# henriChevreux/distillation_trajectories

Measured on AMD Instinct MI355X. Metric: trajectory-timesteps/sec (B×T U-Net fwd) at 16×16 T=50, higher is better.
Workload: dtype f32 (fp32-accurate; convolutions: exact 3-plane bf16 operand split on bf16 MFMA with fp32 accumulate, or native fp32 MFMA, chosen per layer)

## Files before the change

distillation_trajectories_amd/csrc/dt_conv_strip.hip:

```cpp
#include <mutex>
#include <type_traits>

#include "dt_conv_epilogue.h"

namespace dt {

extern __shared__ __attribute__((aligned(16))) __bf16 strip_lds[];

template <int BM, int BN, int KC = 1, int WK = 1>
__global__ __launch_bounds__(256, KC == 1 ? 3 : 2) void conv_strip_bf16x6_kernel(const ConvParams p) {
  constexpr int WN = WK > 1 ? BN / 64 : (BM == 256 ? 1 : 2), WM = 4 / (WN * WK), NT = 256;
  constexpr int MI = BM / (32 * WM), NI = BN / (32 * WN);
  constexpr int KW = KC / WK;
  static_assert(KC % WK == 0 && MI * 32 * WM == BM && NI * 32 * WN == BN && (WK == 1 || (MI == 2 && NI == 2)), "wave layout");
  constexpr int PLANE_B = BN * 16, STAGE_B = 3 * PLANE_B;
  constexpr int AP = BM == 256 ? 3 : (KC == 4 ? 1 : 2);
  const int halo = strip_halo(p.W, BM);
  const int R = BM + 2 * halo;
  const int RZ = (R + 7) & ~7;
  const int PLANE_A = (RZ + 8) * 16;
  __bf16 *As = strip_lds;
  __bf16 *Bs = strip_lds + KC * 3 * PLANE_A;

  const int tid = threadIdx.x, lane = tid & 63;
  const int wave = __builtin_amdgcn_readfirstlane(tid >> 6);
  const int wk = wave % WK, wm = (wave / WK) / WN, wn = (wave / WK) % WN;
  const int half = lane >> 5, l31 = lane & 31;
  const int m0 = blockIdx.x * BM, n0 = blockIdx.y * BN;
  const int HW = p.H * p.W;
  const int CC = p.cin_p >> 4;

  bool s_in[AP], s_ok[AP], s_core[AP];
  int s_off[AP], s_off2[AP], s_offb[AP], s_lds[AP];
#pragma unroll
  for (int i = 0; i < AP; ++i) {
    const int item = tid + i * NT;
    const int srow = item >> 1, hh = item & 1;
    const int m = m0 - halo + srow;
    s_in[i] = item < 2 * R;
    s_ok[i] = s_in[i] && m >= 0 && m < p.M;
    s_core[i] = s_ok[i] && srow >= halo && srow < halo + BM;
    const int mm = s_ok[i] ? m : 0;
    s_off[i] = mm * p.cin_p + hh * 8;
    s_off2[i] = mm * p.cin2_p + hh * 8;
    s_offb[i] = mm * p.b_stride + hh * 8;
    s_lds[i] = srow * 16 + ((hh ^ ((srow >> 3) & 1)) << 3);
  }
  constexpr bool B_ALL = WK > 1 && BN * 4 == NT;
  constexpr int NB = B_ALL ? KC * 3 / 2 : KC * 3, SB = B_ALL ? 2 : 1;
  static_assert(!B_ALL || (KC * 3) % 2 == 0, "weight staging");
  const bool b_thread = B_ALL || tid < BN * 2;
  const int bt = B_ALL ? (tid & (BN * 2 - 1)) : tid, bsub = B_ALL ? tid / (BN * 2) : 0;
  const size_t w_plane = (size_t)p.n_p * 16;
  const __bf16 *wbase = reinterpret_cast<const __bf16 *>(p.w) + (size_t)n0 * 16 + bt * 8 + bsub * w_plane;
  const __bf16 *wbase2 = reinterpret_cast<const __bf16 *>(p.w2) + (size_t)n0 * 16 + bt * 8 + bsub * w_plane;
  const int b_lds = bsub * PLANE_B + bt * 8;

  int a_row[MI];
  unsigned a_mask[MI];
#pragma unroll
  for (int mi = 0; mi < MI; ++mi) {
    const int row_i = wm * (MI * 32) + mi * 32 + l31;
    const int m = m0 + row_i;
    a_row[mi] = row_i + halo;
    unsigned mask = 0;
    if (m < p.M) {
      const int rem = m % HW;
      const int y = rem / p.W, x = rem - y * p.W;
#pragma unroll
      for (int t = 0; t < 9; ++t) {
        const int yy = y + t / 3 - 1, xx = x + t % 3 - 1;
        if (yy >= 0 && yy < p.H && xx >= 0 && xx < p.W) mask |= 1u << t;
      }
    }
    a_mask[mi] = mask;
  }
  int b_frag[NI];
#pragma unroll
  for (int ni = 0; ni < NI; ++ni) {
    const int row = wn * (NI * 32) + ni * 32 + l31;
    b_frag[ni] = row * 16 + ((half ^ ((row >> 3) & 1)) << 3);
  }

  f32x16 acc[MI][NI];
#pragma unroll
  for (int mi = 0; mi < MI; ++mi)
#pragma unroll
    for (int ni = 0; ni < NI; ++ni)
#pragma unroll
      for (int r = 0; r < 16; ++r) acc[mi][ni][r] = 0.f;

  const int n_main = (CC + p.splits * KC - 1) / (p.splits * KC);
  const int cc0 = blockIdx.z * n_main * KC;
  const int CC2 = p.cin2_p >> 4;
  const int n_chunks = n_main + (p.in2 ? (CC2 + KC - 1) / KC : 0);

  f32x4 sa0[KC][AP], sa1[KC][AP];
  u32x4 rb[NB];
  auto load_strip = [&](int ch) __attribute__((always_inline)) {
#pragma unroll
    for (int kk = 0; kk < KC; ++kk)
#pragma unroll
    for (int i = 0; i < AP; ++i) {
      sa0[kk][i] = f32x4{0.f, 0.f, 0.f, 0.f}; sa1[kk][i] = sa0[kk][i];
      if (ch < n_main) {
        const int cc = cc0 + ch * KC + kk;
        if (s_ok[i] && cc < CC) {
          const float *src = (p.in_b && cc >= p.cc_a) ? p.in_b + s_offb[i] + (cc - p.cc_a) * 16 : p.in + s_off[i] + cc * 16;
          sa0[kk][i] = *reinterpret_cast<const f32x4 *>(src);
          sa1[kk][i] = *reinterpret_cast<const f32x4 *>(src + 4);
        }
      } else if (s_core[i] && (ch - n_main) * KC + kk < CC2) {
        const int c2 = (ch - n_main) * KC + kk;
        const float *src = (p.in2_b && c2 >= p.cc_a) ? p.in2_b + s_offb[i] + (c2 - p.cc_a) * 16 : p.in2 + s_off2[i] + c2 * 16;
        sa0[kk][i] = *reinterpret_cast<const f32x4 *>(src);
        sa1[kk][i] = *reinterpret_cast<const f32x4 *>(src + 4);
      }
    }
  };
  auto write_strip = [&]() __attribute__((always_inline)) {
#pragma unroll
    for (int kk = 0; kk < KC; ++kk)
#pragma unroll
    for (int i = 0; i < AP; ++i)
      if (s_in[i]) {
        bf16x8 p1, p2, p3;
        split8(sa0[kk][i], sa1[kk][i], p1, p2, p3);
        __bf16 *A = As + kk * 3 * PLANE_A;
        *reinterpret_cast<bf16x8 *>(A + s_lds[i]) = p1;
        *reinterpret_cast<bf16x8 *>(A + PLANE_A + s_lds[i]) = p2;
        *reinterpret_cast<bf16x8 *>(A + 2 * PLANE_A + s_lds[i]) = p3;
      }
  };
  const size_t tap_stride = (size_t)p.ccw * 3 * w_plane, group_stride = (size_t)KC * 3 * w_plane;
  const __bf16 *wrun = wbase + (size_t)cc0 * 3 * w_plane;
  enum { ADV_NONE = 0, ADV_TAP, ADV_GROUP, ADV_SKIP0, ADV_SKIP };
  auto load_b = [&](int adv) __attribute__((always_inline)) {
    if (adv == ADV_TAP) wrun += tap_stride;
    else if (adv == ADV_GROUP) wrun = wrun - 8 * tap_stride + group_stride;
    else if (adv == ADV_SKIP0) wrun = wbase2;
    else if (adv == ADV_SKIP) wrun += group_stride;
    if (b_thread) {
#pragma unroll
      for (int i = 0; i < NB; ++i)
        rb[i] = *reinterpret_cast<const u32x4 *>(wrun + (SB * i) * w_plane);
    }
  };
  auto write_b = [&](int stage) __attribute__((always_inline)) {
    if (b_thread) {
      __bf16 *B = Bs + stage * KC * STAGE_B;
#pragma unroll
      for (int i = 0; i < NB; ++i) *reinterpret_cast<u32x4 *>(B + (SB * i) * PLANE_B + b_lds) = rb[i];
    }
  };

  constexpr bool DB = WK > 1;
  bf16x8 fbn[KW][NI][3];
  auto load_bd = [&](int adv) __attribute__((always_inline)) {
    if (adv == ADV_TAP) wrun += tap_stride;
    else if (adv == ADV_GROUP) wrun = wrun - 8 * tap_stride + group_stride;
    else if (adv == ADV_SKIP0) wrun = wbase2;
    else if (adv == ADV_SKIP) wrun += group_stride;
    const __bf16 *wt = wrun - (bt * 8 + bsub * w_plane);
#pragma unroll
    for (int kw = 0; kw < KW; ++kw)
#pragma unroll
      for (int ni = 0; ni < NI; ++ni)
#pragma unroll
        for (int pl = 0; pl < 3; ++pl)
          fbn[kw][ni][pl] = *reinterpret_cast<const bf16x8 *>(wt + ((wk * KW + kw) * 3 + pl) * w_plane + b_frag[ni]);
  };

  load_strip(0);
  if (DB) load_bd(ADV_NONE); else load_b(ADV_NONE);
  if (tid < 48 * KC) *reinterpret_cast<u32x4 *>(As + (tid >> 4) * PLANE_A + RZ * 16 + (tid & 15) * 8) = u32x4{0u, 0u, 0u, 0u};
  write_strip();
  if (!DB) write_b(0);
  __syncthreads();

  int step = 0;
  bool stage_next_strip = true;
  auto do_step = [&](auto TT, int ch, bool first_tap, bool last_tap, bool next_chunk, int adv) __attribute__((always_inline)) {
    constexpr int tt = decltype(TT)::value;
    const bool more = !last_tap || next_chunk;
    if (first_tap && next_chunk && stage_next_strip) load_strip(ch + 1);
    bf16x8 fbc[KW][NI][3];
    if (DB) {
#pragma unroll
      for (int kw = 0; kw < KW; ++kw)
#pragma unroll
        for (int ni = 0; ni < NI; ++ni)
#pragma unroll
          for (int pl = 0; pl < 3; ++pl) fbc[kw][ni][pl] = fbn[kw][ni][pl];
      if (more) load_bd(adv);
    } else if (more) load_b(adv);
    {
      int wv = p.W;
      asm volatile("" : "+s"(wv));
      const int shift = (tt / 3 - 1) * wv + (tt % 3 - 1);
      int a_e[MI];
#pragma unroll
      for (int mi = 0; mi < MI; ++mi) {
        int row0 = a_row[mi];
        asm volatile("" : "+v"(row0));
        const int srow = row0 + shift;
        const int lrow = ((a_mask[mi] >> tt) & 1u) ? srow : RZ + (srow & 7);
        a_e[mi] = lrow * 16 + ((half ^ ((srow >> 3) & 1)) << 3);
      }
#pragma unroll
      for (int kw = 0; kw < KW; ++kw) {
        const int kk = wk * KW + kw;
        const __bf16 *A = As + kk * 3 * PLANE_A;
        const __bf16 *B = Bs + ((step & 1) * KC + kk) * STAGE_B;
        bf16x8 fb[NI][3];
#pragma unroll
        for (int ni = 0; ni < NI; ++ni)
#pragma unroll
          for (int pl = 0; pl < 3; ++pl)
            fb[ni][pl] = DB ? fbc[kw][ni][pl] : *reinterpret_cast<const bf16x8 *>(B + pl * PLANE_B + b_frag[ni]);
#pragma unroll
        for (int mi = 0; mi < MI; ++mi) {
          bf16x8 fa[3];
#pragma unroll
          for (int pl = 0; pl < 3; ++pl)
            fa[pl] = *reinterpret_cast<const bf16x8 *>(A + pl * PLANE_A + a_e[mi]);
#pragma unroll
          for (int ni = 0; ni < NI; ++ni) {
            f32x16 c = acc[mi][ni];
            c = __builtin_amdgcn_mfma_f32_32x32x16_bf16(fa[2], fb[ni][0], c, 0, 0, 0);
            c = __builtin_amdgcn_mfma_f32_32x32x16_bf16(fa[1], fb[ni][1], c, 0, 0, 0);
            c = __builtin_amdgcn_mfma_f32_32x32x16_bf16(fa[0], fb[ni][2], c, 0, 0, 0);
            c = __builtin_amdgcn_mfma_f32_32x32x16_bf16(fa[1], fb[ni][0], c, 0, 0, 0);
            c = __builtin_amdgcn_mfma_f32_32x32x16_bf16(fa[0], fb[ni][1], c, 0, 0, 0);
            c = __builtin_amdgcn_mfma_f32_32x32x16_bf16(fa[0], fb[ni][0], c, 0, 0, 0);
            acc[mi][ni] = c;
          }
        }
      }
    }
    if (!DB && more) write_b((step + 1) & 1);
    const bool restage = last_tap && next_chunk && stage_next_strip;
    if (restage) {
      __syncthreads();
      write_strip();
    }
    if (!DB || restage) __syncthreads();
    ++step;
  };

  constexpr bool DIRECT = MI * KW <= 2 && KC >= 2;
  f32x4 ga0[KW][MI][2], ga1[KW][MI][2];
  const int n_skip = p.in2 ? (CC2 + KC - 1) / KC : 0;
  auto load_a = [&](f32x4 (&g)[KW][MI][2], int s2) __attribute__((always_inline)) {
#pragma unroll
    for (int kw = 0; kw < KW; ++kw)
#pragma unroll
      for (int mi = 0; mi < MI; ++mi) {
        const int c2 = s2 * KC + wk * KW + kw;
        const int m = m0 + wm * (MI * 32) + mi * 32 + l31;
        g[kw][mi][0] = f32x4{0.f, 0.f, 0.f, 0.f}; g[kw][mi][1] = g[kw][mi][0];
        if (m < p.M && c2 < CC2) {
          const float *src = (p.in2_b && c2 >= p.cc_a) ? p.in2_b + (size_t)m * p.b_stride + (c2 - p.cc_a) * 16 + half * 8
                                                       : p.in2 + (size_t)m * p.cin2_p + c2 * 16 + half * 8;
          g[kw][mi][0] = *reinterpret_cast<const f32x4 *>(src);
          g[kw][mi][1] = *reinterpret_cast<const f32x4 *>(src + 4);
        }
      }
  };
  auto skip_step = [&](f32x4 (&g)[KW][MI][2], int s2) __attribute__((always_inline)) {
    const bool more = s2 + 1 < n_skip;
    bf16x8 fbc[KW][NI][3];
    if (DB) {
#pragma unroll
      for (int kw = 0; kw < KW; ++kw)
#pragma unroll
        for (int ni = 0; ni < NI; ++ni)
#pragma unroll
          for (int pl = 0; pl < 3; ++pl) fbc[kw][ni][pl] = fbn[kw][ni][pl];
      if (more) load_bd(ADV_SKIP);
    } else if (more) load_b(ADV_SKIP);
#pragma unroll
    for (int kw = 0; kw < KW; ++kw) {
      const int kk = wk * KW + kw;
      const __bf16 *B = Bs + ((step & 1) * KC + kk) * STAGE_B;
      bf16x8 fb[NI][3];
#pragma unroll
      for (int ni = 0; ni < NI; ++ni)
#pragma unroll
        for (int pl = 0; pl < 3; ++pl) fb[ni][pl] = DB ? fbc[kw][ni][pl] : *reinterpret_cast<const bf16x8 *>(B + pl * PLANE_B + b_frag[ni]);
#pragma unroll
      for (int mi = 0; mi < MI; ++mi) {
        bf16x8 fa[3];
        split8(g[kw][mi][0], g[kw][mi][1], fa[0], fa[1], fa[2]);
#pragma unroll
        for (int ni = 0; ni < NI; ++ni) {
          f32x16 c = acc[mi][ni];
          c = __builtin_amdgcn_mfma_f32_32x32x16_bf16(fa[2], fb[ni][0], c, 0, 0, 0);
          c = __builtin_amdgcn_mfma_f32_32x32x16_bf16(fa[1], fb[ni][1], c, 0, 0, 0);
          c = __builtin_amdgcn_mfma_f32_32x32x16_bf16(fa[0], fb[ni][2], c, 0, 0, 0);
          c = __builtin_amdgcn_mfma_f32_32x32x16_bf16(fa[1], fb[ni][0], c, 0, 0, 0);
          c = __builtin_amdgcn_mfma_f32_32x32x16_bf16(fa[0], fb[ni][1], c, 0, 0, 0);
          c = __builtin_amdgcn_mfma_f32_32x32x16_bf16(fa[0], fb[ni][0], c, 0, 0, 0);
          acc[mi][ni] = c;
        }
      }
    }
    if (s2 + 2 < n_skip) load_a(g, s2 + 2);
    if (!DB) {
      if (more) write_b((step + 1) & 1);
      __syncthreads();
    }
    ++step;
  };

  const int prio_grp = ((blockIdx.x + gridDim.x * (blockIdx.y + gridDim.y * blockIdx.z)) >> 8) & 1;
  const bool use_prio = gridDim.x * gridDim.y * gridDim.z <= 512;
  for (int ch = 0; ch < n_main; ++ch) {
    if (use_prio) {
      if ((ch ^ prio_grp) & 1) __builtin_amdgcn_s_setprio(1);
      else __builtin_amdgcn_s_setprio(0);
    }
    const bool next_chunk = ch + 1 < ((WK > 1 && p.in2) ? n_main : n_chunks);
    if (DIRECT && WK == 1 && p.in2 && ch + 1 == n_main) {
      stage_next_strip = false;
      load_a(ga0, 0);
      if (n_skip > 1) load_a(ga1, 1);
    }
    do_step(std::integral_constant<int, 0>{}, ch, true, false, next_chunk, ADV_TAP);
    do_step(std::integral_constant<int, 1>{}, ch, false, false, next_chunk, ADV_TAP);
    do_step(std::integral_constant<int, 2>{}, ch, false, false, next_chunk, ADV_TAP);
    do_step(std::integral_constant<int, 3>{}, ch, false, false, next_chunk, ADV_TAP);
    do_step(std::integral_constant<int, 4>{}, ch, false, false, next_chunk, ADV_TAP);
    do_step(std::integral_constant<int, 5>{}, ch, false, false, next_chunk, ADV_TAP);
    do_step(std::integral_constant<int, 6>{}, ch, false, false, next_chunk, ADV_TAP);
    do_step(std::integral_constant<int, 7>{}, ch, false, false, next_chunk, ADV_TAP);
    do_step(std::integral_constant<int, 8>{}, ch, false, true, next_chunk, ch + 1 < n_main ? ADV_GROUP : ADV_SKIP0);
    if (ch + 1 == n_main && p.in2) {
      if constexpr (WK == 1) {
        conv_midpoint<MI, NI>(p, acc, n0, wn, l31);
      } else {
        constexpr int P = BN + 4, COPY = WM * 32 * P;
        float *red = reinterpret_cast<float *>(strip_lds);
#pragma unroll
        for (int mi = 0; mi < MI; ++mi) {
          if (mi || DB) __syncthreads();
#pragma unroll
          for (int ni = 0; ni < NI; ++ni)
#pragma unroll
            for (int r = 0; r < 16; ++r)
              red[wk * COPY + (wm * 32 + 4 * half + (r & 3) + 8 * (r >> 2)) * P + wn * (NI * 32) + ni * 32 + l31] = acc[mi][ni][r];
          __syncthreads();
#pragma unroll
          for (int ni = 0; ni < NI; ++ni)
#pragma unroll
            for (int r = 0; r < 16; ++r) {
              const float *src = red + (wm * 32 + 4 * half + (r & 3) + 8 * (r >> 2)) * P + wn * (NI * 32) + ni * 32 + l31;
              float v = src[0];
#pragma unroll
              for (int c = 1; c < WK; ++c) v += src[c * COPY];
              acc[mi][ni][r] = wk == 0 ? v : 0.f;
            }
        }
        if (wk == 0) conv_midpoint<MI, NI>(p, acc, n0, wn, l31);
        __syncthreads();
        if (DB) load_bd(ADV_SKIP0); else load_b(ADV_SKIP0);
        if (DIRECT) {
          load_a(ga0, 0);
          if (n_skip > 1) load_a(ga1, 1);
        } else {
          load_strip(n_main);
          if (tid < 48 * KC) *reinterpret_cast<u32x4 *>(As + (tid >> 4) * PLANE_A + RZ * 16 + (tid & 15) * 8) = u32x4{0u, 0u, 0u, 0u};
          write_strip();
        }
        if (!DB) write_b(step & 1);
        __syncthreads();
      }
    }
  }
  __builtin_amdgcn_s_setprio(0);
  if (DIRECT) {
    for (int s2 = 0; s2 < n_skip; s2 += 2) {
      skip_step(ga0, s2);
      if (s2 + 1 < n_skip) skip_step(ga1, s2 + 1);
    }
  } else {
    for (int ch = n_main; ch < n_chunks; ++ch)
      do_step(std::integral_constant<int, 4>{}, ch, true, true, ch + 1 < n_chunks, ADV_SKIP);
  }
  conv_epilogue<MI, NI, WM, WK>(p, acc, reinterpret_cast<float *>(strip_lds), m0, n0, wm, wn, half, l31, wk);
}

int launch_conv_strip(const ConvParams &p_in, hipStream_t s) {
  ConvParams p = p_in;
  const int bm = p.bm, bn = p.bn, kind = p.kind;
  const int kc = strip_kc(kind, bm, bn);
  dim3 grid((p.M + bm - 1) / bm, p.n_p / bn, p.splits);
  size_t lds = strip_lds_bytes(p.W, bm, bn, kind);
  p.dup_stage2 = 0;
  if (p.n_dup == 2 && p.pool_out) {
    const size_t rows1 = bm == 256 || kc == 4 || (kind == KIND_STRIPK && bm == 128) ? 128 : 64;
    const size_t rows2 = bm == 256 ? 128 : (bm == 128 ? 64 : 32);
    const size_t need = (rows1 + (kind == KIND_STRIPK ? rows2 : rows1)) * (bn + 4) * sizeof(float);
    if (need <= strip_lds_limit(kind)) {
      p.dup_stage2 = 1;
      if (need > lds) lds = need;
    }
  }
  if (kind != KIND_STRIP) {
    static std::once_flag attr_once;
    static int attr_status = DT_OK;
    std::call_once(attr_once, [] {
      const void *fns[8] = {reinterpret_cast<const void *>(&conv_strip_bf16x6_kernel<64, 128, 2, 2>),
                            reinterpret_cast<const void *>(&conv_strip_bf16x6_kernel<64, 64, 4, 4>),
                            reinterpret_cast<const void *>(&conv_strip_bf16x6_kernel<128, 64, 2, 2>),
                            reinterpret_cast<const void *>(&conv_strip_bf16x6_kernel<256, 64, 2>),
                            reinterpret_cast<const void *>(&conv_strip_bf16x6_kernel<128, 128, 2>),
                            reinterpret_cast<const void *>(&conv_strip_bf16x6_kernel<128, 64, 2>),
                            reinterpret_cast<const void *>(&conv_strip_bf16x6_kernel<64, 128, 2>),
                            reinterpret_cast<const void *>(&conv_strip_bf16x6_kernel<64, 64, 2>)};
      for (const void *f : fns) {
        const hipError_t e = hipFuncSetAttribute(f, hipFuncAttributeMaxDynamicSharedMemorySize, 98304);
        if (e != hipSuccess) attr_status = (int)e;
      }
    });
    if (attr_status != DT_OK) return attr_status;
    if (kind == KIND_STRIPK && bn == 128) conv_strip_bf16x6_kernel<64, 128, 2, 2><<<grid, 256, lds, s>>>(p);
    else if (kind == KIND_STRIPK && bm == 64) conv_strip_bf16x6_kernel<64, 64, 4, 4><<<grid, 256, lds, s>>>(p);
    else if (kind == KIND_STRIPK) conv_strip_bf16x6_kernel<128, 64, 2, 2><<<grid, 256, lds, s>>>(p);
    else if (bm == 256) conv_strip_bf16x6_kernel<256, 64, 2><<<grid, 256, lds, s>>>(p);
    else if (bm == 128 && bn == 128) conv_strip_bf16x6_kernel<128, 128, 2><<<grid, 256, lds, s>>>(p);
    else if (bm == 128) conv_strip_bf16x6_kernel<128, 64, 2><<<grid, 256, lds, s>>>(p);
    else if (bn == 128) conv_strip_bf16x6_kernel<64, 128, 2><<<grid, 256, lds, s>>>(p);
    else conv_strip_bf16x6_kernel<64, 64, 2><<<grid, 256, lds, s>>>(p);
    DT_LAUNCH_CHECK();
    return DT_OK;
  }
  if (bm == 256) conv_strip_bf16x6_kernel<256, 64><<<grid, 256, lds, s>>>(p);
  else if (bm == 128 && bn == 128) conv_strip_bf16x6_kernel<128, 128><<<grid, 256, lds, s>>>(p);
  else if (bm == 128) conv_strip_bf16x6_kernel<128, 64><<<grid, 256, lds, s>>>(p);
  else if (bn == 128) conv_strip_bf16x6_kernel<64, 128><<<grid, 256, lds, s>>>(p);
  else conv_strip_bf16x6_kernel<64, 64><<<grid, 256, lds, s>>>(p);
  DT_LAUNCH_CHECK();
  return DT_OK;
}

}
```

Before: 355,800.

## Specialize strip conv kernel on skip input and prefetch weights two taps ahead

Adds a compile-time SKIP template flag so launches without a second (skip) input compile out the skip-path registers, offsets and branches, and dispatch picks the specialization at launch. For the split-K direct-weight path without skip input, weight fragments are now kept in a three-slot rotating register buffer and loaded two taps ahead instead of one. The deeper prefetch is meant to hide global-load latency behind MFMA work. In exchange it raises register pressure and doubles the number of kernel instantiations.

```diff
diff --git a/distillation_trajectories_amd/csrc/dt_conv_strip.hip b/distillation_trajectories_amd/csrc/dt_conv_strip.hip
--- a/distillation_trajectories_amd/csrc/dt_conv_strip.hip
+++ b/distillation_trajectories_amd/csrc/dt_conv_strip.hip
@@ -7,7 +7,7 @@
 
 extern __shared__ __attribute__((aligned(16))) __bf16 strip_lds[];
 
-template <int BM, int BN, int KC = 1, int WK = 1>
+template <int BM, int BN, int KC, int WK, bool SKIP>
 __global__ __launch_bounds__(256, KC == 1 ? 3 : 2) void conv_strip_bf16x6_kernel(const ConvParams p) {
   constexpr int WN = WK > 1 ? BN / 64 : (BM == 256 ? 1 : 2), WM = 4 / (WN * WK), NT = 256;
   constexpr int MI = BM / (32 * WM), NI = BN / (32 * WN);
@@ -30,8 +30,10 @@
   const int HW = p.H * p.W;
   const int CC = p.cin_p >> 4;
 
-  bool s_in[AP], s_ok[AP], s_core[AP];
-  int s_off[AP], s_off2[AP], s_offb[AP], s_lds[AP];
+  bool s_in[AP], s_ok[AP];
+  int s_off[AP], s_offb[AP], s_lds[AP];
+  [[maybe_unused]] bool s_core[SKIP ? AP : 1];
+  [[maybe_unused]] int s_off2[SKIP ? AP : 1];
 #pragma unroll
   for (int i = 0; i < AP; ++i) {
     const int item = tid + i * NT;
@@ -39,10 +41,12 @@
     const int m = m0 - halo + srow;
     s_in[i] = item < 2 * R;
     s_ok[i] = s_in[i] && m >= 0 && m < p.M;
-    s_core[i] = s_ok[i] && srow >= halo && srow < halo + BM;
     const int mm = s_ok[i] ? m : 0;
     s_off[i] = mm * p.cin_p + hh * 8;
-    s_off2[i] = mm * p.cin2_p + hh * 8;
+    if constexpr (SKIP) {
+      s_core[i] = s_ok[i] && srow >= halo && srow < halo + BM;
+      s_off2[i] = mm * p.cin2_p + hh * 8;
+    }
     s_offb[i] = mm * p.b_stride + hh * 8;
     s_lds[i] = srow * 16 + ((hh ^ ((srow >> 3) & 1)) << 3);
   }
@@ -53,7 +57,8 @@
   const int bt = B_ALL ? (tid & (BN * 2 - 1)) : tid, bsub = B_ALL ? tid / (BN * 2) : 0;
   const size_t w_plane = (size_t)p.n_p * 16;
   const __bf16 *wbase = reinterpret_cast<const __bf16 *>(p.w) + (size_t)n0 * 16 + bt * 8 + bsub * w_plane;
-  const __bf16 *wbase2 = reinterpret_cast<const __bf16 *>(p.w2) + (size_t)n0 * 16 + bt * 8 + bsub * w_plane;
+  [[maybe_unused]] const __bf16 *wbase2 = nullptr;
+  if constexpr (SKIP) wbase2 = reinterpret_cast<const __bf16 *>(p.w2) + (size_t)n0 * 16 + bt * 8 + bsub * w_plane;
   const int b_lds = bsub * PLANE_B + bt * 8;
 
   int a_row[MI];
@@ -92,8 +97,12 @@
 
   const int n_main = (CC + p.splits * KC - 1) / (p.splits * KC);
   const int cc0 = blockIdx.z * n_main * KC;
-  const int CC2 = p.cin2_p >> 4;
-  const int n_chunks = n_main + (p.in2 ? (CC2 + KC - 1) / KC : 0);
+  [[maybe_unused]] int CC2 = 0, n_skip = 0;
+  if constexpr (SKIP) {
+    CC2 = p.cin2_p >> 4;
+    n_skip = p.in2 ? (CC2 + KC - 1) / KC : 0;
+  }
+  const int n_chunks = n_main + n_skip;
 
   f32x4 sa0[KC][AP], sa1[KC][AP];
   u32x4 rb[NB];
@@ -103,18 +112,22 @@
 #pragma unroll
     for (int i = 0; i < AP; ++i) {
       sa0[kk][i] = f32x4{0.f, 0.f, 0.f, 0.f}; sa1[kk][i] = sa0[kk][i];
-      if (ch < n_main) {
+      bool main_chunk = true;
+      if constexpr (SKIP) main_chunk = ch < n_main;
+      if (main_chunk) {
         const int cc = cc0 + ch * KC + kk;
         if (s_ok[i] && cc < CC) {
           const float *src = (p.in_b && cc >= p.cc_a) ? p.in_b + s_offb[i] + (cc - p.cc_a) * 16 : p.in + s_off[i] + cc * 16;
           sa0[kk][i] = *reinterpret_cast<const f32x4 *>(src);
           sa1[kk][i] = *reinterpret_cast<const f32x4 *>(src + 4);
         }
-      } else if (s_core[i] && (ch - n_main) * KC + kk < CC2) {
-        const int c2 = (ch - n_main) * KC + kk;
-        const float *src = (p.in2_b && c2 >= p.cc_a) ? p.in2_b + s_offb[i] + (c2 - p.cc_a) * 16 : p.in2 + s_off2[i] + c2 * 16;
-        sa0[kk][i] = *reinterpret_cast<const f32x4 *>(src);
-        sa1[kk][i] = *reinterpret_cast<const f32x4 *>(src + 4);
+      } else if constexpr (SKIP) {
+        if (s_core[i] && (ch - n_main) * KC + kk < CC2) {
+          const int c2 = (ch - n_main) * KC + kk;
+          const float *src = (p.in2_b && c2 >= p.cc_a) ? p.in2_b + s_offb[i] + (c2 - p.cc_a) * 16 : p.in2 + s_off2[i] + c2 * 16;
+          sa0[kk][i] = *reinterpret_cast<const f32x4 *>(src);
+          sa1[kk][i] = *reinterpret_cast<const f32x4 *>(src + 4);
+        }
       }
     }
   };
@@ -135,11 +148,16 @@
   const size_t tap_stride = (size_t)p.ccw * 3 * w_plane, group_stride = (size_t)KC * 3 * w_plane;
   const __bf16 *wrun = wbase + (size_t)cc0 * 3 * w_plane;
   enum { ADV_NONE = 0, ADV_TAP, ADV_GROUP, ADV_SKIP0, ADV_SKIP };
-  auto load_b = [&](int adv) __attribute__((always_inline)) {
+  auto advance = [&](int adv) __attribute__((always_inline)) {
     if (adv == ADV_TAP) wrun += tap_stride;
     else if (adv == ADV_GROUP) wrun = wrun - 8 * tap_stride + group_stride;
-    else if (adv == ADV_SKIP0) wrun = wbase2;
-    else if (adv == ADV_SKIP) wrun += group_stride;
+    if constexpr (SKIP) {
+      if (adv == ADV_SKIP0) wrun = wbase2;
+      else if (adv == ADV_SKIP) wrun += group_stride;
+    }
+  };
+  auto load_b = [&](int adv) __attribute__((always_inline)) {
+    advance(adv);
     if (b_thread) {
 #pragma unroll
       for (int i = 0; i < NB; ++i)
@@ -155,12 +173,11 @@
   };
 
   constexpr bool DB = WK > 1;
-  bf16x8 fbn[KW][NI][3];
-  auto load_bd = [&](int adv) __attribute__((always_inline)) {
-    if (adv == ADV_TAP) wrun += tap_stride;
-    else if (adv == ADV_GROUP) wrun = wrun - 8 * tap_stride + group_stride;
-    else if (adv == ADV_SKIP0) wrun = wbase2;
-    else if (adv == ADV_SKIP) wrun += group_stride;
+  constexpr bool AHEAD2 = DB && !SKIP;
+  bf16x8 fbr[AHEAD2 ? 3 : 1][KW][NI][3];
+  bf16x8 (&fbn)[KW][NI][3] = fbr[0];
+  auto load_bd = [&](bf16x8 (&dst)[KW][NI][3], int adv) __attribute__((always_inline)) {
+    advance(adv);
     const __bf16 *wt = wrun - (bt * 8 + bsub * w_plane);
 #pragma unroll
     for (int kw = 0; kw < KW; ++kw)
@@ -168,11 +185,12 @@
       for (int ni = 0; ni < NI; ++ni)
 #pragma unroll
         for (int pl = 0; pl < 3; ++pl)
-          fbn[kw][ni][pl] = *reinterpret_cast<const bf16x8 *>(wt + ((wk * KW + kw) * 3 + pl) * w_plane + b_frag[ni]);
+          dst[kw][ni][pl] = *reinterpret_cast<const bf16x8 *>(wt + ((wk * KW + kw) * 3 + pl) * w_plane + b_frag[ni]);
   };
 
   load_strip(0);
-  if (DB) load_bd(ADV_NONE); else load_b(ADV_NONE);
+  if (DB) load_bd(fbn, ADV_NONE); else load_b(ADV_NONE);
+  if constexpr (AHEAD2) load_bd(fbr[1], ADV_TAP);
   if (tid < 48 * KC) *reinterpret_cast<u32x4 *>(As + (tid >> 4) * PLANE_A + RZ * 16 + (tid & 15) * 8) = u32x4{0u, 0u, 0u, 0u};
   write_strip();
   if (!DB) write_b(0);
@@ -185,14 +203,16 @@
     const bool more = !last_tap || next_chunk;
     if (first_tap && next_chunk && stage_next_strip) load_strip(ch + 1);
     bf16x8 fbc[KW][NI][3];
-    if (DB) {
+    if constexpr (AHEAD2) {
+      if (tt < 7 || next_chunk) load_bd(fbr[(tt + 2) % 3], tt == 7 ? ADV_GROUP : ADV_TAP);
+    } else if (DB) {
 #pragma unroll
       for (int kw = 0; kw < KW; ++kw)
 #pragma unroll
         for (int ni = 0; ni < NI; ++ni)
 #pragma unroll
           for (int pl = 0; pl < 3; ++pl) fbc[kw][ni][pl] = fbn[kw][ni][pl];
-      if (more) load_bd(adv);
+      if (more) load_bd(fbn, adv);
     } else if (more) load_b(adv);
     {
       int wv = p.W;
@@ -217,7 +237,7 @@
         for (int ni = 0; ni < NI; ++ni)
 #pragma unroll
           for (int pl = 0; pl < 3; ++pl)
-            fb[ni][pl] = DB ? fbc[kw][ni][pl] : *reinterpret_cast<const bf16x8 *>(B + pl * PLANE_B + b_frag[ni]);
+            fb[ni][pl] = AHEAD2 ? fbr[AHEAD2 ? tt % 3 : 0][kw][ni][pl] : DB ? fbc[kw][ni][pl] : *reinterpret_cast<const bf16x8 *>(B + pl * PLANE_B + b_frag[ni]);
 #pragma unroll
         for (int mi = 0; mi < MI; ++mi) {
           bf16x8 fa[3];
@@ -248,10 +268,11 @@
     ++step;
   };
 
-  constexpr bool DIRECT = MI * KW <= 2 && KC >= 2;
-  f32x4 ga0[KW][MI][2], ga1[KW][MI][2];
-  const int n_skip = p.in2 ? (CC2 + KC - 1) / KC : 0;
-  auto load_a = [&](f32x4 (&g)[KW][MI][2], int s2) __attribute__((always_inline)) {
+  constexpr bool DIRECT = SKIP && MI * KW <= 2 && KC >= 2;
+  struct no_regs {};
+  using skip_regs = std::conditional_t<SKIP, f32x4[KW][MI][2], no_regs>;
+  [[maybe_unused]] skip_regs ga0, ga1;
+  auto load_a = [&](auto &g, int s2) __attribute__((always_inline)) {
 #pragma unroll
     for (int kw = 0; kw < KW; ++kw)
 #pragma unroll
@@ -267,7 +288,7 @@
         }
       }
   };
-  auto skip_step = [&](f32x4 (&g)[KW][MI][2], int s2) __attribute__((always_inline)) {
+  auto skip_step = [&](auto &g, int s2) __attribute__((always_inline)) {
     const bool more = s2 + 1 < n_skip;
     bf16x8 fbc[KW][NI][3];
     if (DB) {
@@ -277,7 +298,7 @@
         for (int ni = 0; ni < NI; ++ni)
 #pragma unroll
           for (int pl = 0; pl < 3; ++pl) fbc[kw][ni][pl] = fbn[kw][ni][pl];
-      if (more) load_bd(ADV_SKIP);
+      if (more) load_bd(fbn, ADV_SKIP);
     } else if (more) load_b(ADV_SKIP);
 #pragma unroll
     for (int kw = 0; kw < KW; ++kw) {
@@ -320,11 +341,14 @@
       if ((ch ^ prio_grp) & 1) __builtin_amdgcn_s_setprio(1);
       else __builtin_amdgcn_s_setprio(0);
     }
-    const bool next_chunk = ch + 1 < ((WK > 1 && p.in2) ? n_main : n_chunks);
-    if (DIRECT && WK == 1 && p.in2 && ch + 1 == n_main) {
-      stage_next_strip = false;
-      load_a(ga0, 0);
-      if (n_skip > 1) load_a(ga1, 1);
+    bool next_chunk = ch + 1 < n_main;
+    if constexpr (SKIP) next_chunk = ch + 1 < ((WK > 1 && p.in2) ? n_main : n_chunks);
+    if constexpr (DIRECT && WK == 1) {
+      if (p.in2 && ch + 1 == n_main) {
+        stage_next_strip = false;
+        load_a(ga0, 0);
+        if (n_skip > 1) load_a(ga1, 1);
+      }
     }
     do_step(std::integral_constant<int, 0>{}, ch, true, false, next_chunk, ADV_TAP);
     do_step(std::integral_constant<int, 1>{}, ch, false, false, next_chunk, ADV_TAP);
@@ -334,8 +358,8 @@
     do_step(std::integral_constant<int, 5>{}, ch, false, false, next_chunk, ADV_TAP);
     do_step(std::integral_constant<int, 6>{}, ch, false, false, next_chunk, ADV_TAP);
     do_step(std::integral_constant<int, 7>{}, ch, false, false, next_chunk, ADV_TAP);
-    do_step(std::integral_constant<int, 8>{}, ch, false, true, next_chunk, ch + 1 < n_main ? ADV_GROUP : ADV_SKIP0);
-    if (ch + 1 == n_main && p.in2) {
+    do_step(std::integral_constant<int, 8>{}, ch, false, true, next_chunk, !SKIP || ch + 1 < n_main ? ADV_GROUP : ADV_SKIP0);
+    if constexpr (SKIP) if (ch + 1 == n_main && p.in2) {
       if constexpr (WK == 1) {
         conv_midpoint<MI, NI>(p, acc, n0, wn, l31);
       } else {
@@ -363,8 +387,8 @@
         }
         if (wk == 0) conv_midpoint<MI, NI>(p, acc, n0, wn, l31);
         __syncthreads();
-        if (DB) load_bd(ADV_SKIP0); else load_b(ADV_SKIP0);
-        if (DIRECT) {
+        if (DB) load_bd(fbn, ADV_SKIP0); else load_b(ADV_SKIP0);
+        if constexpr (DIRECT) {
           load_a(ga0, 0);
           if (n_skip > 1) load_a(ga1, 1);
         } else {
@@ -378,16 +402,31 @@
     }
   }
   __builtin_amdgcn_s_setprio(0);
-  if (DIRECT) {
+  if constexpr (DIRECT) {
     for (int s2 = 0; s2 < n_skip; s2 += 2) {
       skip_step(ga0, s2);
       if (s2 + 1 < n_skip) skip_step(ga1, s2 + 1);
     }
-  } else {
+  } else if constexpr (SKIP) {
     for (int ch = n_main; ch < n_chunks; ++ch)
       do_step(std::integral_constant<int, 4>{}, ch, true, true, ch + 1 < n_chunks, ADV_SKIP);
   }
   conv_epilogue<MI, NI, WM, WK>(p, acc, reinterpret_cast<float *>(strip_lds), m0, n0, wm, wn, half, l31, wk);
+}
+
+template <int BM, int BN, int KC, int WK>
+static hipError_t strip_allow_lds() {
+  const hipError_t e = hipFuncSetAttribute(reinterpret_cast<const void *>(&conv_strip_bf16x6_kernel<BM, BN, KC, WK, false>),
+                                           hipFuncAttributeMaxDynamicSharedMemorySize, 98304);
+  if (e != hipSuccess) return e;
+  return hipFuncSetAttribute(reinterpret_cast<const void *>(&conv_strip_bf16x6_kernel<BM, BN, KC, WK, true>),
+                             hipFuncAttributeMaxDynamicSharedMemorySize, 98304);
+}
+
+template <int BM, int BN, int KC = 1, int WK = 1>
+static void strip_launch(const ConvParams &p, dim3 grid, size_t lds, hipStream_t s) {
+  if (p.in2) conv_strip_bf16x6_kernel<BM, BN, KC, WK, true><<<grid, 256, lds, s>>>(p);
+  else conv_strip_bf16x6_kernel<BM, BN, KC, WK, false><<<grid, 256, lds, s>>>(p);
 }
 
 int launch_conv_strip(const ConvParams &p_in, hipStream_t s) {
@@ -410,36 +449,29 @@
     static std::once_flag attr_once;
     static int attr_status = DT_OK;
     std::call_once(attr_once, [] {
-      const void *fns[8] = {reinterpret_cast<const void *>(&conv_strip_bf16x6_kernel<64, 128, 2, 2>),
-                            reinterpret_cast<const void *>(&conv_strip_bf16x6_kernel<64, 64, 4, 4>),
-                            reinterpret_cast<const void *>(&conv_strip_bf16x6_kernel<128, 64, 2, 2>),
-                            reinterpret_cast<const void *>(&conv_strip_bf16x6_kernel<256, 64, 2>),
-                            reinterpret_cast<const void *>(&conv_strip_bf16x6_kernel<128, 128, 2>),
-                            reinterpret_cast<const void *>(&conv_strip_bf16x6_kernel<128, 64, 2>),
-                            reinterpret_cast<const void *>(&conv_strip_bf16x6_kernel<64, 128, 2>),
-                            reinterpret_cast<const void *>(&conv_strip_bf16x6_kernel<64, 64, 2>)};
-      for (const void *f : fns) {
-        const hipError_t e = hipFuncSetAttribute(f, hipFuncAttributeMaxDynamicSharedMemorySize, 98304);
+      const hipError_t es[8] = {strip_allow_lds<64, 128, 2, 2>(), strip_allow_lds<64, 64, 4, 4>(), strip_allow_lds<128, 64, 2, 2>(),
+                                strip_allow_lds<256, 64, 2, 1>(), strip_allow_lds<128, 128, 2, 1>(), strip_allow_lds<128, 64, 2, 1>(),
+                                strip_allow_lds<64, 128, 2, 1>(), strip_allow_lds<64, 64, 2, 1>()};
+      for (const hipError_t e : es)
         if (e != hipSuccess) attr_status = (int)e;
-      }
     });
     if (attr_status != DT_OK) return attr_status;
-    if (kind == KIND_STRIPK && bn == 128) conv_strip_bf16x6_kernel<64, 128, 2, 2><<<grid, 256, lds, s>>>(p);
-    else if (kind == KIND_STRIPK && bm == 64) conv_strip_bf16x6_kernel<64, 64, 4, 4><<<grid, 256, lds, s>>>(p);
-    else if (kind == KIND_STRIPK) conv_strip_bf16x6_kernel<128, 64, 2, 2><<<grid, 256, lds, s>>>(p);
-    else if (bm == 256) conv_strip_bf16x6_kernel<256, 64, 2><<<grid, 256, lds, s>>>(p);
-    else if (bm == 128 && bn == 128) conv_strip_bf16x6_kernel<128, 128, 2><<<grid, 256, lds, s>>>(p);
-    else if (bm == 128) conv_strip_bf16x6_kernel<128, 64, 2><<<grid, 256, lds, s>>>(p);
-    else if (bn == 128) conv_strip_bf16x6_kernel<64, 128, 2><<<grid, 256, lds, s>>>(p);
-    else conv_strip_bf16x6_kernel<64, 64, 2><<<grid, 256, lds, s>>>(p);
+    if (kind == KIND_STRIPK && bn == 128) strip_launch<64, 128, 2, 2>(p, grid, lds, s);
+    else if (kind == KIND_STRIPK && bm == 64) strip_launch<64, 64, 4, 4>(p, grid, lds, s);
+    else if (kind == KIND_STRIPK) strip_launch<128, 64, 2, 2>(p, grid, lds, s);
+    else if (bm == 256) strip_launch<256, 64, 2>(p, grid, lds, s);
+    else if (bm == 128 && bn == 128) strip_launch<128, 128, 2>(p, grid, lds, s);
+    else if (bm == 128) strip_launch<128, 64, 2>(p, grid, lds, s);
+    else if (bn == 128) strip_launch<64, 128, 2>(p, grid, lds, s);
+    else strip_launch<64, 64, 2>(p, grid, lds, s);
     DT_LAUNCH_CHECK();
     return DT_OK;
   }
-  if (bm == 256) conv_strip_bf16x6_kernel<256, 64><<<grid, 256, lds, s>>>(p);
-  else if (bm == 128 && bn == 128) conv_strip_bf16x6_kernel<128, 128><<<grid, 256, lds, s>>>(p);
-  else if (bm == 128) conv_strip_bf16x6_kernel<128, 64><<<grid, 256, lds, s>>>(p);
-  else if (bn == 128) conv_strip_bf16x6_kernel<64, 128><<<grid, 256, lds, s>>>(p);
-  else conv_strip_bf16x6_kernel<64, 64><<<grid, 256, lds, s>>>(p);
+  if (bm == 256) strip_launch<256, 64>(p, grid, lds, s);
+  else if (bm == 128 && bn == 128) strip_launch<128, 128>(p, grid, lds, s);
+  else if (bm == 128) strip_launch<128, 64>(p, grid, lds, s);
+  else if (bn == 128) strip_launch<64, 128>(p, grid, lds, s);
+  else strip_launch<64, 64>(p, grid, lds, s);
   DT_LAUNCH_CHECK();
   return DT_OK;
 }
```

Result: no change. 359,300, median of 6 (+1.0%).
